# argumentcomputer/multi-stark

Hardware: NVIDIA B200
Metric: lde_merkle_gelem_per_s (higher is better)
Workload: dtype u64

## Files before the change

multi_stark_b200/csrc/fri.cu:

```cuda
#include "capi_common.hpp"
#include "mmcs.hpp"
#include "blake3.cuh"
#include <algorithm>
#include <cstring>
#include <memory>

namespace msg {

__device__ __forceinline__ u64 fp_inv_d(u64 x) {
    auto sqn = [](u64 v, int n) { for (int i = 0; i < n; i++) v = gl::mul(v, v); return v; };
    u64 t2 = gl::mul(sqn(x, 1), x);
    u64 t4 = gl::mul(sqn(t2, 2), t2);
    u64 t8 = gl::mul(sqn(t4, 4), t4);
    u64 t16 = gl::mul(sqn(t8, 8), t8);
    u64 t24 = gl::mul(sqn(t16, 8), t8);
    u64 t28 = gl::mul(sqn(t24, 4), t4);
    u64 t30 = gl::mul(sqn(t28, 2), t2);
    u64 t31 = gl::mul(sqn(t30, 1), x);
    u64 a = sqn(t31, 1);
    u64 b = gl::mul(a, x);
    return gl::mul(sqn(a, 32), b);
}
__device__ __forceinline__ gl::e2 e2_inverse_d(gl::e2 x) {
    u64 norm = gl::sub(gl::sqr(x.a), gl::mul7(gl::sqr(x.b)));
    u64 ni = fp_inv_d(norm);
    return gl::e2_make(gl::mul(x.a, ni), gl::mul(gl::neg(x.b), ni));
}

constexpr int kInvPerThread = 8;
__global__ void __launch_bounds__(256) k_inv_denoms(u64* invden, u32 log_h, gl::e2 z, gl::PowTable xtab, u64 row0, u64 len) {
    const u64 H = len;
    u64 i0 = ((u64)blockIdx.x * blockDim.x + threadIdx.x) * kInvPerThread;
    if (i0 >= H) return;
    const int cnt = (int)min((u64)kInvPerThread, H - i0);
    u64 va[kInvPerThread];
    gl::e2 pref[kInvPerThread];
    gl::e2 acc = gl::e2_make(1, 0);
#pragma unroll
    for (int k = 0; k < kInvPerThread; k++) {
        pref[k] = acc;
        va[k] = 0;
        if (k < cnt) {
            u64 x = gl::pow_lookup(xtab, gl::rev_bits((u32)(row0 + i0 + k), log_h));
            va[k] = gl::sub(z.a, x);
            acc = gl::e2_mul(acc, gl::e2_make(va[k], z.b));
        }
    }
    gl::e2 inv = e2_inverse_d(acc);
#pragma unroll
    for (int k = kInvPerThread - 1; k >= 0; k--) {
        if (k < cnt) {
            gl::e2 r = gl::e2_mul(inv, pref[k]);
            inv = gl::e2_mul(inv, gl::e2_make(va[k], z.b));
            invden[2 * (i0 + k)] = r.a;
            invden[2 * (i0 + k) + 1] = r.b;
        }
    }
}

constexpr int kMaxPts = 4;
struct BaryParams {
    const u64* M;
    const u64* invden[kMaxPts];
    u64* partial;
    u64 h;
    u32 w, c0, wc;
    u32 rows_per_step, tile_rows;
};
__host__ __device__ __forceinline__ size_t bary_dd_offset(u32 tile_rows, u32 wc) { return ((size_t)tile_rows * wc + 1) & ~(size_t)1; }
template <int NPTS>
__global__ void __launch_bounds__(256) k_bary_partial(BaryParams p) {
    extern __shared__ __align__(16) u64 sm_b[];
    const u32 t = threadIdx.x;
    const u32 TR = p.tile_rows, wc = p.wc;
    u64* tile = sm_b;
    ulonglong2* dd = reinterpret_cast<ulonglong2*>(sm_b + bary_dd_offset(TR, wc));
    const u32 active = p.rows_per_step * wc;
    const u32 c = t % wc, lane_row = t / wc;
    gl::Acc160 acc[2 * NPTS];
#pragma unroll
    for (int k = 0; k < 2 * NPTS; k++) acc[k] = gl::acc_zero();
// ... 897 lines not shown
```

multi_stark_b200/csrc/gl.cuh:

```cuda
#pragma once
#include <cstdint>
#include <cuda_runtime.h>

typedef unsigned long long u64;
typedef unsigned int u32;

#define GLD_P 0xFFFFFFFF00000001ull
#define GLD_EPS 0xFFFFFFFFull

namespace gl {


__device__ __forceinline__ u64 pack(u32 lo, u32 hi) { return ((u64)hi << 32) | lo; }

__device__ __forceinline__ u64 canon(u64 x) {
    u32 x0 = (u32)x, x1 = (u32)(x >> 32), r0, r1;
    asm("{\n\t"
        ".reg .u32 t, k;\n\t"
        "add.cc.u32 t, %2, 0xffffffff;\n\t"
        "addc.cc.u32 t, %3, 0;\n\t"
        "addc.u32 k, 0, 0;\n\t"
        "neg.s32 k, k;\n\t"
        "add.cc.u32 %0, %2, k;\n\t"
        "addc.u32 %1, %3, 0;\n\t"
// ... 39 lines not shown

__device__ __forceinline__ u64 reduce128_lazy(u64 lo, u64 hi) {
    u32 l0 = (u32)lo, l1 = (u32)(lo >> 32), hl = (u32)hi, hh = (u32)(hi >> 32), r0, r1;
    asm("{\n\t"
        ".reg .u32 m, k, t0, t1;\n\t"
        "sub.cc.u32 %0, %2, %5;\n\t"
        "subc.cc.u32 %1, %3, 0;\n\t"
        "subc.u32 m, 0, 0;\n\t"
        "sub.cc.u32 %0, %0, m;\n\t"
        "subc.u32 %1, %1, 0;\n\t"
        "sub.cc.u32 t0, 0, %4;\n\t"
        "subc.u32 t1, %4, 0;\n\t"
        "add.cc.u32 %0, %0, t0;\n\t"
        "addc.cc.u32 %1, %1, t1;\n\t"
        "addc.u32 k, 0, 0;\n\t"
        "neg.s32 k, k;\n\t"
        "add.cc.u32 %0, %0, k;\n\t"
        "addc.u32 %1, %1, 0;\n\t"
        "}"
        : "=&r"(r0), "=&r"(r1)
        : "r"(l0), "r"(l1), "r"(hl), "r"(hh));
    return pack(r0, r1);
}
namespace gf {
__device__ __forceinline__ u64 reduce128(u64 lo, u64 hi);
}
__device__ __forceinline__ u64 mul(u64 a, u64 b) {
    unsigned __int128 pr = (unsigned __int128)a * b;
    return gf::reduce128((u64)pr, (u64)(pr >> 64));
}
__device__ __forceinline__ u64 mul_lazy(u64 a, u64 b) { return reduce128_lazy(a * b, __umul64hi(a, b)); }
__device__ __forceinline__ u64 sqr(u64 a) { return mul(a, a); }

__device__ __forceinline__ u64 pow(u64 a, u64 e) {
    u64 acc = 1;
    while (e) {
        if (e & 1) acc = mul(acc, a);
        a = sqr(a);
        e >>= 1;
    }
    return acc;
}
__device__ __forceinline__ u64 inv(u64 a) { return pow(a, GLD_P - 2); }
__device__ __forceinline__ u64 halve(u64 a) { return (a & 1) ? (a >> 1) + (GLD_P >> 1) + 1 : a >> 1; }

namespace gf {
__device__ __forceinline__ u64 sub(u64 a, u64 b) { return sub_lazy(a, b); }
__device__ __forceinline__ u64 add(u64 a, u64 b) { return sub_lazy(a, GLD_P - b); }
__device__ __forceinline__ u64 reduce128(u64 lo, u64 hi) {
    u32 l0 = (u32)lo, l1 = (u32)(lo >> 32), h0 = (u32)hi, h1 = (u32)(hi >> 32);
    u64 r;
    asm("{\n\t"
        ".reg .u32 t0, t1, m, k, z, r0, r1;\n\t"
        ".reg .u64 rr;\n\t"
        "sub.cc.u32 t0, %1, %4;\n\t"
        "subc.cc.u32 t1, %2, 0;\n\t"
        "subc.u32 m, 0, 0;\n\t"
        "sub.cc.u32 t0, t0, m;\n\t"
        "subc.u32 t1, t1, 0;\n\t"
        "mad.lo.cc.u32 r0, %3, 0xffffffff, t0;\n\t"
        "madc.hi.cc.u32 r1, %3, 0xffffffff, t1;\n\t"
        "addc.u32 k, 0, 0;\n\t"
        "mov.b64 rr, {r0, r1};\n\t"
        "mad.wide.u32 rr, k, 0xffffffff, rr;\n\t"
        "mov.b64 {r0, r1}, rr;\n\t"
        "add.cc.u32 z, r0, 0xffffffff;\n\t"
        "addc.cc.u32 z, r1, 0;\n\t"
        "addc.u32 k, 0, 0;\n\t"
        "mad.wide.u32 %0, k, 0xffffffff, rr;\n\t"
        "}"
        : "=l"(r)
        : "r"(l0), "r"(l1), "r"(h0), "r"(h1));
    return r;
}
__device__ __forceinline__ u64 mul(u64 a, u64 b) {
    unsigned __int128 pr = (unsigned __int128)a * b;
// ... 36 lines not shown
        "mad.lo.cc.u32 %1, %5, %8, %1;\n\t"
        "madc.hi.cc.u32 %2, %5, %8, %2;\n\t"
        "addc.cc.u32 %3, %3, 0;\n\t"
        "addc.u32 %4, %4, 0;\n\t"
        "mad.lo.cc.u32 %1, %6, %7, %1;\n\t"
        "madc.hi.cc.u32 %2, %6, %7, %2;\n\t"
        "addc.cc.u32 %3, %3, 0;\n\t"
        "addc.u32 %4, %4, 0;\n\t"
        "}"
        : "+r"(s.l0), "+r"(s.l1), "+r"(s.l2), "+r"(s.l3), "+r"(s.l4)
        : "r"(a0), "r"(a1), "r"(b0), "r"(b1));
}
__device__ __forceinline__ u64 acc_reduce(const Acc160& s) {
    u64 r = gf::reduce128(pack(s.l0, s.l1), pack(s.l2, s.l3));
    return sub_lazy(r, (u64)s.l4 << 32);
}

struct e2 {
    u64 a, b;
};
__device__ __forceinline__ e2 e2_make(u64 a, u64 b) { e2 r; r.a = a; r.b = b; return r; }
__device__ __forceinline__ e2 e2_add(e2 x, e2 y) { return e2_make(add(x.a, y.a), add(x.b, y.b)); }
__device__ __forceinline__ e2 e2_sub(e2 x, e2 y) { return e2_make(sub(x.a, y.a), sub(x.b, y.b)); }
__device__ __forceinline__ u64 mul7(u64 x) {
    u64 x2 = add(x, x), x4 = add(x2, x2);
    return sub(add(x4, x4), x);
}
__device__ __forceinline__ e2 e2_mul(e2 x, e2 y) {
    u64 v0 = mul(x.a, y.a), v1 = mul(x.b, y.b);
    u64 cross = sub(sub(mul(add(x.a, x.b), add(y.a, y.b)), v0), v1);
    return e2_make(add(v0, mul7(v1)), cross);
}
__device__ __forceinline__ e2 e2_mul_base(e2 x, u64 s) { return e2_make(mul(x.a, s), mul(x.b, s)); }
__device__ __forceinline__ e2 e2_inv(e2 x) {
    u64 norm = sub(sqr(x.a), mul7(sqr(x.b)));
    u64 ni = inv(norm);
    return e2_make(mul(x.a, ni), mul(neg(x.b), ni));
}

struct PowTable {
    const u64* lo;
    const u64* hi;
    u32 h1;
};
__device__ __forceinline__ u64 pow_lookup(const PowTable& t, u64 e) {
    return mul(__ldg(t.hi + (e >> t.h1)), __ldg(t.lo + (e & ((1ull << t.h1) - 1))));
}

__device__ __forceinline__ u32 rev_bits(u32 x, u32 bits) { return bits ? (__brev(x) >> (32 - bits)) : 0u; }

}
```

multi_stark_b200/csrc/quotient.cu:

```cuda
#include "capi_common.hpp"
#include <cstdio>
#include <cstdlib>
#include "../host/blake3_host.hpp"
#include <cstring>
#include "mmcs.hpp"
#include "lowering.hpp"
#include <algorithm>
#include <cstring>

namespace msg {

}

struct msgpu_program {
    msg::Ctx* ctx = nullptr;
    msg::Instr* d_full = nullptr;
    msg::Instr* d_prefix = nullptr;
    u32 n_full = 0, n_prefix = 0, slots_full = 0, slots_prefix = 0;
    u32 n_zeros = 0, n_lookups = 0, n_args = 0;
    u32* d_zero_slots = nullptr;
    u32 *d_mult_full = nullptr, *d_args_full = nullptr;
    u32 *d_mult_prefix = nullptr, *d_args_prefix = nullptr;
    u32* d_arg_off = nullptr;
    u32 pre_width = 0, main_width = 0, stage2_width = 0;
    std::vector<void*> owned;
};

namespace msg {

__device__ __forceinline__ gl::e2 e2_mul_k(gl::e2 x, gl::e2 y) { return gl::e2_mul(x, y); }

__device__ __forceinline__ u64 fp_inv(u64 x) {
    auto sqn = [](u64 v, int n) { for (int i = 0; i < n; i++) v = gl::mul(v, v); return v; };
    u64 t2 = gl::mul(sqn(x, 1), x);
    u64 t4 = gl::mul(sqn(t2, 2), t2);
    u64 t8 = gl::mul(sqn(t4, 4), t4);
    u64 t16 = gl::mul(sqn(t8, 8), t8);
    u64 t24 = gl::mul(sqn(t16, 8), t8);
    u64 t28 = gl::mul(sqn(t24, 4), t4);
    u64 t30 = gl::mul(sqn(t28, 2), t2);
    u64 t31 = gl::mul(sqn(t30, 1), x);
    u64 a = sqn(t31, 1);
    u64 b = gl::mul(a, x);
    return gl::mul(sqn(a, 32), b);
}
__device__ __forceinline__ gl::e2 e2_inverse(gl::e2 x) {
    u64 norm = gl::sub(gl::sqr(x.a), gl::mul7(gl::sqr(x.b)));
    u64 ni = fp_inv(norm);
    return gl::e2_make(gl::mul(x.a, ni), gl::mul(gl::neg(x.b), ni));
}

struct RowCtx {
    const u64* rows[3][2];
    const u64* publics;
    u64 first, last, trans;
};

constexpr int kInterpThreads = 128;
constexpr int kSmemSlotsMax = 128;
template <int NSLOT, bool SMEM>
struct Slots;
template <int NSLOT>
struct Slots<NSLOT, false> {
    u64 v[NSLOT];
    __device__ __forceinline__ Slots() {}
    __device__ __forceinline__ u64& operator[](u32 k) { return v[k]; }
};
template <int NSLOT>
struct Slots<NSLOT, true> {
    u64* base;
    __device__ __forceinline__ Slots() {
        extern __shared__ u64 sm_slots[];
        base = sm_slots + threadIdx.x;
    }
    __device__ __forceinline__ u64& operator[](u32 k) { return base[(size_t)k * kInterpThreads]; }
};
template <int NSLOT>
constexpr size_t slots_smem_bytes() { return NSLOT <= kSmemSlotsMax ? (size_t)NSLOT * kInterpThreads * 8 : 0; }

struct NoRoots {
    __device__ __forceinline__ void operator()(u32, u64) const {}
};
template <int NSLOT, class S, class Root = NoRoots>
// ... 29 lines not shown
        }
        slots[dst] = v;
    }
}

struct SelParams {
    gl::PowTable xtab;
    const u64* zh;
    u64 g_inv;
    u64* first;
    u64* last;
    u32 log_nq, log_q;
};
constexpr int kSelPerThread = 4;
__global__ void __launch_bounds__(256) k_selectors(SelParams p) {
    const u64 nq = 1ull << p.log_nq;
    u64 s0 = ((u64)blockIdx.x * blockDim.x + threadIdx.x) * kSelPerThread;
    if (s0 >= nq) return;
    u64 den[2 * kSelPerThread], pref[2 * kSelPerThread], zh[kSelPerThread];
    int cnt = 0;
#pragma unroll
    for (int k = 0; k < kSelPerThread; k++) {
        u64 s = s0 + k;
        if (s >= nq) break;
        u64 i = gl::rev_bits((u32)s, p.log_nq);
        u64 x = gl::pow_lookup(p.xtab, i);
        den[2 * k] = gl::sub(x, 1);
        den[2 * k + 1] = gl::sub(x, p.g_inv);
        zh[k] = p.zh[i & ((1ull << p.log_q) - 1)];
        cnt = k + 1;
    }
    u64 acc = 1;
    for (int k = 0; k < 2 * cnt; k++) { pref[k] = acc; acc = gl::mul(acc, den[k]); }
    u64 inv = fp_inv(acc);
    for (int k = 2 * cnt; k-- > 0;) {
        u64 d = den[k];
        den[k] = gl::mul(inv, pref[k]);
        inv = gl::mul(inv, d);
    }
    for (int k = 0; k < cnt; k++) {
        p.first[s0 + k] = gl::mul(zh[k], den[2 * k]);
        p.last[s0 + k] = gl::mul(zh[k], den[2 * k + 1]);
    }
}

struct QuotParams {
    const Instr* prog;
    const u32* zero_slots;
    const u32 *lk_mult, *lk_argoff, *lk_args;
    const u64 *pre, *s1, *s2;
    const u64* apow;
    const u64 *sel_first, *sel_last, *inv_zh;
    u64* out;
    const u64 *pre_n, *s1_n, *s2_n;
    u32 wn[3], cn[3];
    u64 row0, n_local, next_row0;
    u32 out_stored;
    gl::PowTable xtab;
    u64 publics[8];
    u64 delta[2];
    u64 g_inv;
    u32 n_instr, n_zeros, n_lookups;
    u32 wpre, w1, w2;
    u32 log_nq, log_q;
};

template <int NSLOT>
// ... 37 lines not shown
        fold(gl::add(gl::sub(s2n[1], s2c[1]), inj.b));
    } else {
        for (u32 j = 0; j < p.n_lookups; j++) {
            gl::e2 source = gl::e2_make(s2c[2 * j], s2c[2 * j + 1]);
            gl::e2 target = j + 1 < p.n_lookups ? gl::e2_make(s2c[2 * j + 2], s2c[2 * j + 3])
                                                : gl::e2_make(gl::add(s2n[0], inj.a), gl::add(s2n[1], inj.b));
            gl::e2 f = gl::e2_make(0, 0);
            for (u32 k = p.lk_argoff[j + 1]; k-- > p.lk_argoff[j];) {
                f = gl::e2_mul(f, gamma);
                f.a = gl::add(f.a, slots[p.lk_args[k]]);
            }
            gl::e2 c = gl::e2_mul(gl::e2_add(f, beta), gl::e2_sub(target, source));
            fold(gl::sub(c.a, slots[p.lk_mult[j]]));
            fold(c.b);
        }
    }
    const u64 iv = p.inv_zh[i & ((1ull << p.log_q) - 1)];
    const u64 o = p.out_stored ? sl : i;
    p.out[2 * o] = gl::mul(gl::acc_reduce(fa0), iv);
    p.out[2 * o + 1] = gl::mul(gl::acc_reduce(fa1), iv);
}

__global__ void k_quotient_slices(const u64* S, u64* out, u32 log_big, u32 log_n, u32 d, const u64* weights) {
    const u64 big = 1ull << log_big, n = 1ull << log_n, q = big >> log_n;
    u64 t = (u64)blockIdx.x * blockDim.x + threadIdx.x;
    if (t >= big) return;
    u64 r = t / q, k = t % q;
    u64 j = k * n + r;
    u64 src = gl::rev_bits((u32)((big - j) & (big - 1)), log_big);
    u64 w = weights[k];
    for (u32 c = 0; c < d; c++) out[r * (q * d) + k * d + c] = gl::mul(S[src * d + c], w);
}

struct MsgParams {
    const Instr* prog;
    const u32 *lk_mult, *lk_argoff, *lk_args;
    const u64 *pre, *main;
    u64* msgs;
    u64* mults;
    u64 rows;
    u64 beta[2], gamma[2];
    u32 n_instr, n_lookups, wpre, wmain;
};
template <int NSLOT>
__global__ void __launch_bounds__(128) k_lookup_messages(MsgParams p) {
    const u64 r = (u64)blockIdx.x * blockDim.x + threadIdx.x;
    if (r >= p.rows) return;
    const u64 rn = r + 1 == p.rows ? 0 : r + 1;
    RowCtx cx;
    cx.rows[0][0] = p.pre + r * p.wpre;
    cx.rows[0][1] = p.pre + rn * p.wpre;
    cx.rows[1][0] = p.main + r * p.wmain;
    cx.rows[1][1] = p.main + rn * p.wmain;
    cx.rows[2][0] = cx.rows[2][1] = nullptr;
    cx.publics = nullptr;
    cx.first = r == 0;
    cx.last = r + 1 == p.rows;
    cx.trans = r + 1 != p.rows;
    Slots<NSLOT, (NSLOT <= kSmemSlotsMax)> slots;
    run_program<NSLOT>(p.prog, p.n_instr, slots, cx);
    const gl::e2 beta = gl::e2_make(p.beta[0], p.beta[1]), gamma = gl::e2_make(p.gamma[0], p.gamma[1]);
    for (u32 j = 0; j < p.n_lookups; j++) {
        gl::e2 f = gl::e2_make(0, 0);
        for (u32 k = p.lk_argoff[j + 1]; k-- > p.lk_argoff[j];) {
            f = gl::e2_mul(f, gamma);
            f.a = gl::add(f.a, slots[p.lk_args[k]]);
        }
        f = gl::e2_add(f, beta);
        u64 idx = r * p.n_lookups + j;
        p.msgs[2 * idx] = f.a;
        p.msgs[2 * idx + 1] = f.b;
        p.mults[idx] = slots[p.lk_mult[j]];
    }
}

constexpr int kScanPerThread = 8;
constexpr int kScanThreads = 256;
constexpr int kScanPerBlock = kScanPerThread * kScanThreads;

__device__ __forceinline__ gl::e2 block_sum(gl::e2 v, gl::e2* sm) {
    for (int off = 16; off > 0; off >>= 1) {
        v.a = gl::add(v.a, __shfl_down_sync(0xffffffffu, v.a, off));
        v.b = gl::add(v.b, __shfl_down_sync(0xffffffffu, v.b, off));
    }
    int lane = threadIdx.x & 31, wid = threadIdx.x >> 5;
    if (lane == 0) sm[wid] = v;
    __syncthreads();
    gl::e2 r = gl::e2_make(0, 0);
    if (threadIdx.x == 0)
        for (int w = 0; w < (int)(blockDim.x >> 5); w++) r = gl::e2_add(r, sm[w]);
    return r;
}

__global__ void __launch_bounds__(kScanThreads) k_terms_and_block_sums(u64* msgs, const u64* mults, u64 total, u64* block_sums) {
    __shared__ gl::e2 sm[kScanThreads / 32];
    u64 i0 = ((u64)blockIdx.x * kScanThreads + threadIdx.x) * kScanPerThread;
    gl::e2 pref[kScanPerThread];
    const int cnt = (int)min((u64)kScanPerThread, total > i0 ? total - i0 : 0);
    gl::e2 acc = gl::e2_make(1, 0);
#pragma unroll
    for (int k = 0; k < kScanPerThread; k++) {
        pref[k] = acc;
        if (k < cnt) acc = gl::e2_mul(acc, gl::e2_make(msgs[2 * (i0 + k)], msgs[2 * (i0 + k) + 1]));
    }
    gl::e2 inv = cnt ? e2_inverse(acc) : acc;
    gl::e2 sum = gl::e2_make(0, 0);
#pragma unroll
    for (int k = kScanPerThread - 1; k >= 0; k--) {
        if (k < cnt) {
            gl::e2 x = gl::e2_make(msgs[2 * (i0 + k)], msgs[2 * (i0 + k) + 1]);
            gl::e2 xi = gl::e2_mul(inv, pref[k]);
            inv = gl::e2_mul(inv, x);
            gl::e2 term = gl::e2_mul_base(xi, mults[i0 + k]);
            msgs[2 * (i0 + k)] = term.a;
            msgs[2 * (i0 + k) + 1] = term.b;
            sum = gl::e2_add(sum, term);
        }
    }
    gl::e2 bs = block_sum(sum, sm);
    if (threadIdx.x == 0) { block_sums[2 * blockIdx.x] = bs.a; block_sums[2 * blockIdx.x + 1] = bs.b; }
}

__global__ void __launch_bounds__(1024) k_scan_block_sums(u64* block_sums, u64 nblocks) {
    __shared__ gl::e2 sm[1024];
    u64 per = (nblocks + blockDim.x - 1) / blockDim.x;
    u64 lo = (u64)threadIdx.x * per, hi = min(nblocks, lo + per);
    gl::e2 s = gl::e2_make(0, 0);
    for (u64 i = lo; i < hi; i++) s = gl::e2_add(s, gl::e2_make(block_sums[2 * i], block_sums[2 * i + 1]));
    sm[threadIdx.x] = s;
    __syncthreads();
    for (int off = 1; off < (int)blockDim.x; off <<= 1) {
        gl::e2 t = sm[threadIdx.x];
        if ((int)threadIdx.x >= off) t = gl::e2_add(t, sm[threadIdx.x - off]);
        __syncthreads();
        sm[threadIdx.x] = t;
        __syncthreads();
    }
    gl::e2 run = threadIdx.x ? sm[threadIdx.x - 1] : gl::e2_make(0, 0);
    for (u64 i = lo; i < hi; i++) {
        gl::e2 v = gl::e2_make(block_sums[2 * i], block_sums[2 * i + 1]);
        block_sums[2 * i] = run.a;
        block_sums[2 * i + 1] = run.b;
        run = gl::e2_add(run, v);
    }
    if (threadIdx.x == blockDim.x - 1) {
        gl::e2 tot = sm[blockDim.x - 1];
        block_sums[2 * nblocks] = tot.a;
        block_sums[2 * nblocks + 1] = tot.b;
    }
}

__global__ void __launch_bounds__(kScanThreads) k_scan_write(const u64* terms, u64 total, const u64* block_offsets, u64* out) {
    __shared__ gl::e2 sm[kScanThreads];
    u64 i0 = ((u64)blockIdx.x * kScanThreads + threadIdx.x) * kScanPerThread;
    gl::e2 v[kScanPerThread];
    gl::e2 s = gl::e2_make(0, 0);
    for (int k = 0; k < kScanPerThread; k++) {
        v[k] = i0 + k < total ? gl::e2_make(terms[2 * (i0 + k)], terms[2 * (i0 + k) + 1]) : gl::e2_make(0, 0);
        s = gl::e2_add(s, v[k]);
    }
    sm[threadIdx.x] = s;
    __syncthreads();
    for (int off = 1; off < kScanThreads; off <<= 1) {
        gl::e2 t = sm[threadIdx.x];
        if ((int)threadIdx.x >= off) t = gl::e2_add(t, sm[threadIdx.x - off]);
        __syncthreads();
        sm[threadIdx.x] = t;
        __syncthreads();
    }
    gl::e2 run = gl::e2_make(block_offsets[2 * blockIdx.x], block_offsets[2 * blockIdx.x + 1]);
    if (threadIdx.x) run = gl::e2_add(run, sm[threadIdx.x - 1]);
    for (int k = 0; k < kScanPerThread; k++) {
        if (i0 + k >= total) break;
        out[2 * (i0 + k)] = run.a;
        out[2 * (i0 + k) + 1] = run.b;
        run = gl::e2_add(run, v[k]);
    }
}

__global__ void __launch_bounds__(kScanThreads) k_claims(const u64* claims, u64 n_claims, u32 len, gl::e2 beta, gl::e2 gamma,
                                                         u64* partial) {
    __shared__ gl::e2 sm[kScanThreads / 32];
    u64 i0 = ((u64)blockIdx.x * kScanThreads + threadIdx.x) * kScanPerThread;
    const int cnt = (int)min((u64)kScanPerThread, n_claims > i0 ? n_claims - i0 : 0);
    gl::e2 v[kScanPerThread], pref[kScanPerThread];
    gl::e2 acc = gl::e2_make(1, 0);
#pragma unroll
    for (int k = 0; k < kScanPerThread; k++) {
        pref[k] = acc;
        v[k] = acc;
        if (k < cnt) {
            const u64* c = claims + (i0 + k) * len;
            gl::e2 f = gl::e2_make(0, 0);
            for (u32 a = len; a-- > 0;) {
                f = gl::e2_mul(f, gamma);
                f.a = gl::add(f.a, c[a]);
            }
            v[k] = gl::e2_add(f, beta);
            acc = gl::e2_mul(acc, v[k]);
        }
    }
    gl::e2 inv = cnt ? e2_inverse(acc) : acc;
    gl::e2 sum = gl::e2_make(0, 0);
#pragma unroll
    for (int k = kScanPerThread - 1; k >= 0; k--) {
        if (k < cnt) {
            sum = gl::e2_add(sum, gl::e2_mul(inv, pref[k]));
            inv = gl::e2_mul(inv, v[k]);
        }
    }
    gl::e2 bs = block_sum(sum, sm);
    if (threadIdx.x == 0) { partial[2 * blockIdx.x] = bs.a; partial[2 * blockIdx.x + 1] = bs.b; }
}

template <class T>
static T* upload_vec(Ctx& c, msgpu_program* prog, const std::vector<T>& v) {
    T* d = nullptr;
    MSG_CUDA(cudaMalloc(&d, std::max<size_t>(v.size(), 1) * sizeof(T)));
    prog->owned.push_back(d);
    if (!v.empty()) MSG_CUDA(cudaMemcpyAsync(d, v.data(), v.size() * sizeof(T), cudaMemcpyHostToDevice, c.stream));
    return d;
}

static msgpu_program* program_create(Ctx& c, const msgpu_graph_desc& g) {
    MSG_REQUIRE(g.lookup_prefix_len <= g.n_nodes, "program: lookup prefix longer than the node vector");
    MSG_REQUIRE(g.stage2_width == 2 * std::max<u32>(g.n_lookups, 1), "program: stage-2 width must be 2 * max(lookups, 1)");
    std::vector<u32> pin_lk, pin_all;
    u32 n_args = g.n_lookups ? g.lookup_arg_off[g.n_lookups] : 0;
    for (u32 j = 0; j < g.n_lookups; j++) pin_lk.push_back(g.lookup_mult[j]);
    for (u32 k = 0; k < n_args; k++) pin_lk.push_back(g.lookup_args[k]);
    pin_all = pin_lk;
    std::vector<u32> roots(g.zeros, g.zeros + g.n_zeros);
    for (u32 p : pin_lk) MSG_REQUIRE(p < g.lookup_prefix_len, "program: lookup node outside the prefix");
    Lowered full, prefix;
    try {
// ... 125 lines not shown
    *ptr = m.ptr;
}

}

using namespace msg;

struct msgpu_claims {
    Ctx* ctx;
    u64* d;
    u64 n, len;
    cudaEvent_t ready = nullptr;
};

namespace msg {
__global__ void __launch_bounds__(256) k_encode_claims(const u64* claims, u64 n_words, u32 len, uint8_t* msg) {
    u64 j = (u64)blockIdx.x * blockDim.x + threadIdx.x;
    if (j >= n_words) return;
    u64 claim = j / (len + 1);
    u32 k = (u32)(j % (len + 1));
    u64 v = k == 0 ? (u64)len : claims[claim * len + (k - 1)];
    uint8_t* o = msg + 8 * j;
#pragma unroll
    for (int b = 0; b < 8; b++) o[b] = (uint8_t)(v >> (8 * b));
}
}

static void claims_sum(Ctx& c, const u64* d_claims, u64 n_claims, u64 claim_len, const uint64_t* beta2, const uint64_t* gamma2,
                       uint64_t* out2) {
    StageScope ss(c, "stage2");
    out2[0] = out2[1] = 0;
    if (n_claims == 0) return;
    u64 nblocks = (n_claims + kScanPerBlock - 1) / kScanPerBlock;
    DevBuf part(c, nblocks * 16);
    {
        KLaunch kl(c, "k_claims");
        k_claims<<<(unsigned)nblocks, kScanThreads, 0, c.stream>>>(d_claims, n_claims, (u32)claim_len, gl::e2{beta2[0], beta2[1]},
                                                                   gl::e2{gamma2[0], gamma2[1]}, part.u());
    }
    MSG_CUDA(cudaGetLastError());
    std::vector<u64> hp(nblocks * 2);
    MSG_CUDA(cudaMemcpyAsync(hp.data(), part.p, nblocks * 16, cudaMemcpyDeviceToHost, c.stream));
    c.sync();
    msh::Fp2 acc;
    for (u64 b = 0; b < nblocks; b++) acc += msh::Fp2(msh::Fp(hp[2 * b]), msh::Fp(hp[2 * b + 1]));
    out2[0] = acc.c[0].v;
    out2[1] = acc.c[1].v;
}

extern "C" {

int msgpu_program_create(msgpu_ctx* h, const msgpu_graph_desc* desc, msgpu_program** out) {
    return guard([&] {
        MSG_REQUIRE(desc && out, "program_create: null argument");
        *out = program_create(h->c, *desc);
    });
}
void msgpu_program_free(msgpu_program* prog) {
    if (!prog) return;
    cudaStreamSynchronize(prog->ctx->stream);
    for (void* p : prog->owned) cudaFree(p);
    delete prog;
}

int msgpu_stage2_trace(msgpu_ctx* h, const msgpu_program* prog, const uint64_t* pre_dev, const uint64_t* main_dev,
                       uint64_t rows, const uint64_t* beta2, const uint64_t* gamma2, uint64_t* stage2_out_dev,
                       uint64_t* local_sum2) {
    return guard([&] {
        Ctx& c = h->c;
        StageScope ss(c, "stage2");
        MSG_REQUIRE(prog && stage2_out_dev && local_sum2, "stage2_trace: null argument");
        MSG_REQUIRE(main_dev || prog->n_lookups == 0, "stage2_trace: the main trace is needed to evaluate the lookups");
        MSG_REQUIRE(prog->pre_width == 0 || pre_dev, "stage2_trace: circuit has a preprocessed trace but none was given");
        local_sum2[0] = local_sum2[1] = 0;
        if (rows == 0) return;
        u32 L = prog->n_lookups;
        if (L == 0) {
            MSG_CUDA(cudaMemsetAsync(stage2_out_dev, 0, rows * 2 * 8, c.stream));
            return;
        }
        u64 total = rows * L;
        u64 nblocks = (total + kScanPerBlock - 1) / kScanPerBlock;
        DevBuf msgs(c, total * 16), mults(c, total * 8), bsums(c, (nblocks + 1) * 16);
        MsgParams mp{};
        mp.prog = prog->d_prefix;
        mp.n_instr = prog->n_prefix;
        mp.lk_mult = prog->d_mult_prefix;
        mp.lk_argoff = prog->d_arg_off;
        mp.lk_args = prog->d_args_prefix;
        mp.pre = (const u64*)pre_dev;
        mp.main = (const u64*)main_dev;
        mp.msgs = msgs.u();
        mp.mults = mults.u();
        mp.rows = rows;
        mp.beta[0] = beta2[0]; mp.beta[1] = beta2[1];
        mp.gamma[0] = gamma2[0]; mp.gamma[1] = gamma2[1];
        mp.n_lookups = L;
        mp.wpre = prog->pre_width;
        mp.wmain = prog->main_width;
        launch_by_slots(prog->slots_prefix, [&](auto ns) {
            KLaunch kl(c, "k_lookup_messages");
            constexpr int NS = decltype(ns)::value;
            constexpr size_t smem = slots_smem_bytes<NS>();
            if (smem > 48 * 1024) ensure_max_smem(k_lookup_messages<NS>, (int)smem);
            k_lookup_messages<NS><<<(unsigned)((rows + 127) / 128), kInterpThreads, smem, c.stream>>>(mp);
        });
        MSG_CUDA(cudaGetLastError());
        {
            KLaunch kl(c, "k_terms_and_block_sums");
            k_terms_and_block_sums<<<(unsigned)nblocks, kScanThreads, 0, c.stream>>>(msgs.u(), mults.u(), total, bsums.u());
        }
        MSG_CUDA(cudaGetLastError());
        {
            KLaunch kl(c, "k_scan_block_sums");
            k_scan_block_sums<<<1, 1024, 0, c.stream>>>(bsums.u(), nblocks);
        }
        MSG_CUDA(cudaGetLastError());
        {
            KLaunch kl(c, "k_scan_write");
            k_scan_write<<<(unsigned)nblocks, kScanThreads, 0, c.stream>>>(msgs.u(), total, bsums.u(), (u64*)stage2_out_dev);
        }
        MSG_CUDA(cudaGetLastError());
        MSG_CUDA(cudaMemcpyAsync(local_sum2, bsums.u() + 2 * nblocks, 16, cudaMemcpyDeviceToHost, c.stream));
        c.sync();
    });
}

int msgpu_claims_accumulator(msgpu_ctx* h, const uint64_t* claims, uint64_t n_claims, uint64_t claim_len,
                             const uint64_t* beta2, const uint64_t* gamma2, uint64_t* out2) {
    return guard([&] {
        Ctx& c = h->c;
        MSG_REQUIRE(claim_len < (1ull << 31), "claims: claim too long");
        DevBuf d(c, n_claims * std::max<u64>(claim_len, 1) * 8);
        if (claim_len && n_claims) MSG_CUDA(cudaMemcpyAsync(d.p, claims, n_claims * claim_len * 8, cudaMemcpyHostToDevice, c.stream));
        claims_sum(c, d.u(), n_claims, claim_len, beta2, gamma2, out2);
    });
}

static void claims_digest(Ctx& c, const u64* d_claims, u64 n_claims, u64 claim_len, const uint8_t* prefix, u64 prefix_len, uint8_t* digest32);

int msgpu_claims_upload(msgpu_ctx* h, const uint64_t* claims, uint64_t n_claims, uint64_t claim_len, const uint8_t* prefix,
                        uint64_t prefix_len, msgpu_claims** out, uint8_t* digest32) {
    return guard([&] {
        Ctx& c = h->c;
        MSG_REQUIRE(out && digest32 && claims && n_claims > 0 && claim_len > 0, "claims_upload: null or empty argument");
        MSG_REQUIRE(claim_len < (1ull << 31) && n_claims <= (~0ull) / 16 / (claim_len + 1), "claims_upload: too large");
        u64 n_vals = n_claims * claim_len;
        DevBuf d(c, n_vals * 8);
        MSG_CUDA(cudaMemcpyAsync(d.p, claims, n_vals * 8, cudaMemcpyHostToDevice, c.stream));
        claims_digest(c, d.u(), n_claims, claim_len, prefix, prefix_len, digest32);
        *out = new msgpu_claims{&c, (u64*)d.release(), n_claims, claim_len};
    });
}

int msgpu_claims_prefetch(msgpu_ctx* h, const uint64_t* claims, uint64_t n_claims, uint64_t claim_len, msgpu_claims** out) {
    return guard([&] {
        Ctx& c = h->c;
// ... 276 lines not shown
```

Before: 27.02.

## Fuse lookup messages and logup inverses, batch inversions across warps

Merges the lookup message kernel and the term/block-sum kernel into one k_logup_terms kernel. It takes the inverse through the base-field norm, with running products stored in the output buffer, so the msgs and mults temporaries go away. Field inversions are batched across a warp with shuffles, so one exponentiation serves 32 threads, with a zero flag for failures. It also rewrites the scan-write as a warp-shuffle scan over spans and unifies the inverse helpers. This adds recomputation of lookup fingerprints and a zero-check readback. The measured LDE/Merkle metric likely only touches k_inv_denoms, via the warp inverse.

After: 27.06, median of 6. Within noise of the previous version (+0.1%).

```diff
diff --git a/multi_stark_b200/csrc/fri.cu b/multi_stark_b200/csrc/fri.cu
--- a/multi_stark_b200/csrc/fri.cu
+++ b/multi_stark_b200/csrc/fri.cu
@@ -7,32 +7,11 @@
 
 namespace msg {
 
-__device__ __forceinline__ u64 fp_inv_d(u64 x) {
-    auto sqn = [](u64 v, int n) { for (int i = 0; i < n; i++) v = gl::mul(v, v); return v; };
-    u64 t2 = gl::mul(sqn(x, 1), x);
-    u64 t4 = gl::mul(sqn(t2, 2), t2);
-    u64 t8 = gl::mul(sqn(t4, 4), t4);
-    u64 t16 = gl::mul(sqn(t8, 8), t8);
-    u64 t24 = gl::mul(sqn(t16, 8), t8);
-    u64 t28 = gl::mul(sqn(t24, 4), t4);
-    u64 t30 = gl::mul(sqn(t28, 2), t2);
-    u64 t31 = gl::mul(sqn(t30, 1), x);
-    u64 a = sqn(t31, 1);
-    u64 b = gl::mul(a, x);
-    return gl::mul(sqn(a, 32), b);
-}
-__device__ __forceinline__ gl::e2 e2_inverse_d(gl::e2 x) {
-    u64 norm = gl::sub(gl::sqr(x.a), gl::mul7(gl::sqr(x.b)));
-    u64 ni = fp_inv_d(norm);
-    return gl::e2_make(gl::mul(x.a, ni), gl::mul(gl::neg(x.b), ni));
-}
-
 constexpr int kInvPerThread = 8;
 __global__ void __launch_bounds__(256) k_inv_denoms(u64* invden, u32 log_h, gl::e2 z, gl::PowTable xtab, u64 row0, u64 len) {
     const u64 H = len;
     u64 i0 = ((u64)blockIdx.x * blockDim.x + threadIdx.x) * kInvPerThread;
-    if (i0 >= H) return;
-    const int cnt = (int)min((u64)kInvPerThread, H - i0);
+    const int cnt = (int)min((u64)kInvPerThread, H > i0 ? H - i0 : 0);
     u64 va[kInvPerThread];
     gl::e2 pref[kInvPerThread];
     gl::e2 acc = gl::e2_make(1, 0);
@@ -46,7 +25,8 @@
             acc = gl::e2_mul(acc, gl::e2_make(va[k], z.b));
         }
     }
-    gl::e2 inv = e2_inverse_d(acc);
+    bool any_zero;
+    gl::e2 inv = gl::e2_inv_warp(acc, any_zero);
 #pragma unroll
     for (int k = kInvPerThread - 1; k >= 0; k--) {
         if (k < cnt) {
diff --git a/multi_stark_b200/csrc/gl.cuh b/multi_stark_b200/csrc/gl.cuh
--- a/multi_stark_b200/csrc/gl.cuh
+++ b/multi_stark_b200/csrc/gl.cuh
@@ -95,16 +95,20 @@
 __device__ __forceinline__ u64 mul_lazy(u64 a, u64 b) { return reduce128_lazy(a * b, __umul64hi(a, b)); }
 __device__ __forceinline__ u64 sqr(u64 a) { return mul(a, a); }
 
-__device__ __forceinline__ u64 pow(u64 a, u64 e) {
-    u64 acc = 1;
-    while (e) {
-        if (e & 1) acc = mul(acc, a);
-        a = sqr(a);
-        e >>= 1;
-    }
-    return acc;
-}
-__device__ __forceinline__ u64 inv(u64 a) { return pow(a, GLD_P - 2); }
+__device__ __forceinline__ u64 inv(u64 x) {
+    auto sqn = [](u64 v, int n) { for (int i = 0; i < n; i++) v = mul(v, v); return v; };
+    u64 t2 = mul(sqn(x, 1), x);
+    u64 t4 = mul(sqn(t2, 2), t2);
+    u64 t8 = mul(sqn(t4, 4), t4);
+    u64 t16 = mul(sqn(t8, 8), t8);
+    u64 t24 = mul(sqn(t16, 8), t8);
+    u64 t28 = mul(sqn(t24, 4), t4);
+    u64 t30 = mul(sqn(t28, 2), t2);
+    u64 t31 = mul(sqn(t30, 1), x);
+    u64 a = sqn(t31, 1);
+    u64 b = mul(a, x);
+    return mul(sqn(a, 32), b);
+}
 __device__ __forceinline__ u64 halve(u64 a) { return (a & 1) ? (a >> 1) + (GLD_P >> 1) + 1 : a >> 1; }
 
 namespace gf {
@@ -207,9 +211,28 @@
     return e2_make(add(v0, mul7(v1)), cross);
 }
 __device__ __forceinline__ e2 e2_mul_base(e2 x, u64 s) { return e2_make(mul(x.a, s), mul(x.b, s)); }
+__device__ __forceinline__ u64 e2_norm(e2 x) { return sub(sqr(x.a), mul7(sqr(x.b))); }
 __device__ __forceinline__ e2 e2_inv(e2 x) {
-    u64 norm = sub(sqr(x.a), mul7(sqr(x.b)));
-    u64 ni = inv(norm);
+    u64 ni = inv(e2_norm(x));
+    return e2_make(mul(x.a, ni), mul(neg(x.b), ni));
+}
+
+__device__ __forceinline__ u64 inv_warp(u64 x, bool& any_zero) {
+    u64 sib[5];
+    u64 g = x;
+#pragma unroll
+    for (int k = 0; k < 5; k++) {
+        sib[k] = __shfl_xor_sync(0xffffffffu, g, 1 << k);
+        g = mul(g, sib[k]);
+    }
+    any_zero = g == 0;
+    u64 gi = inv(g);
+#pragma unroll
+    for (int k = 4; k >= 0; k--) gi = mul(gi, sib[k]);
+    return gi;
+}
+__device__ __forceinline__ e2 e2_inv_warp(e2 x, bool& any_zero) {
+    const u64 ni = inv_warp(e2_norm(x), any_zero);
     return e2_make(mul(x.a, ni), mul(neg(x.b), ni));
 }
 
diff --git a/multi_stark_b200/csrc/quotient.cu b/multi_stark_b200/csrc/quotient.cu
--- a/multi_stark_b200/csrc/quotient.cu
+++ b/multi_stark_b200/csrc/quotient.cu
@@ -29,26 +29,6 @@
 namespace msg {
 
 __device__ __forceinline__ gl::e2 e2_mul_k(gl::e2 x, gl::e2 y) { return gl::e2_mul(x, y); }
-
-__device__ __forceinline__ u64 fp_inv(u64 x) {
-    auto sqn = [](u64 v, int n) { for (int i = 0; i < n; i++) v = gl::mul(v, v); return v; };
-    u64 t2 = gl::mul(sqn(x, 1), x);
-    u64 t4 = gl::mul(sqn(t2, 2), t2);
-    u64 t8 = gl::mul(sqn(t4, 4), t4);
-    u64 t16 = gl::mul(sqn(t8, 8), t8);
-    u64 t24 = gl::mul(sqn(t16, 8), t8);
-    u64 t28 = gl::mul(sqn(t24, 4), t4);
-    u64 t30 = gl::mul(sqn(t28, 2), t2);
-    u64 t31 = gl::mul(sqn(t30, 1), x);
-    u64 a = sqn(t31, 1);
-    u64 b = gl::mul(a, x);
-    return gl::mul(sqn(a, 32), b);
-}
-__device__ __forceinline__ gl::e2 e2_inverse(gl::e2 x) {
-    u64 norm = gl::sub(gl::sqr(x.a), gl::mul7(gl::sqr(x.b)));
-    u64 ni = fp_inv(norm);
-    return gl::e2_make(gl::mul(x.a, ni), gl::mul(gl::neg(x.b), ni));
-}
 
 struct RowCtx {
     const u64* rows[3][2];
@@ -144,7 +124,7 @@
     }
     u64 acc = 1;
     for (int k = 0; k < 2 * cnt; k++) { pref[k] = acc; acc = gl::mul(acc, den[k]); }
-    u64 inv = fp_inv(acc);
+    u64 inv = gl::inv(acc);
     for (int k = 2 * cnt; k-- > 0;) {
         u64 d = den[k];
         den[k] = gl::mul(inv, pref[k]);
@@ -248,48 +228,6 @@
     for (u32 c = 0; c < d; c++) out[r * (q * d) + k * d + c] = gl::mul(S[src * d + c], w);
 }
 
-struct MsgParams {
-    const Instr* prog;
-    const u32 *lk_mult, *lk_argoff, *lk_args;
-    const u64 *pre, *main;
-    u64* msgs;
-    u64* mults;
-    u64 rows;
-    u64 beta[2], gamma[2];
-    u32 n_instr, n_lookups, wpre, wmain;
-};
-template <int NSLOT>
-__global__ void __launch_bounds__(128) k_lookup_messages(MsgParams p) {
-    const u64 r = (u64)blockIdx.x * blockDim.x + threadIdx.x;
-    if (r >= p.rows) return;
-    const u64 rn = r + 1 == p.rows ? 0 : r + 1;
-    RowCtx cx;
-    cx.rows[0][0] = p.pre + r * p.wpre;
-    cx.rows[0][1] = p.pre + rn * p.wpre;
-    cx.rows[1][0] = p.main + r * p.wmain;
-    cx.rows[1][1] = p.main + rn * p.wmain;
-    cx.rows[2][0] = cx.rows[2][1] = nullptr;
-    cx.publics = nullptr;
-    cx.first = r == 0;
-    cx.last = r + 1 == p.rows;
-    cx.trans = r + 1 != p.rows;
-    Slots<NSLOT, (NSLOT <= kSmemSlotsMax)> slots;
-    run_program<NSLOT>(p.prog, p.n_instr, slots, cx);
-    const gl::e2 beta = gl::e2_make(p.beta[0], p.beta[1]), gamma = gl::e2_make(p.gamma[0], p.gamma[1]);
-    for (u32 j = 0; j < p.n_lookups; j++) {
-        gl::e2 f = gl::e2_make(0, 0);
-        for (u32 k = p.lk_argoff[j + 1]; k-- > p.lk_argoff[j];) {
-            f = gl::e2_mul(f, gamma);
-            f.a = gl::add(f.a, slots[p.lk_args[k]]);
-        }
-        f = gl::e2_add(f, beta);
-        u64 idx = r * p.n_lookups + j;
-        p.msgs[2 * idx] = f.a;
-        p.msgs[2 * idx + 1] = f.b;
-        p.mults[idx] = slots[p.lk_mult[j]];
-    }
-}
-
 constexpr int kScanPerThread = 8;
 constexpr int kScanThreads = 256;
 constexpr int kScanPerBlock = kScanPerThread * kScanThreads;
@@ -308,33 +246,84 @@
     return r;
 }
 
-__global__ void __launch_bounds__(kScanThreads) k_terms_and_block_sums(u64* msgs, const u64* mults, u64 total, u64* block_sums) {
-    __shared__ gl::e2 sm[kScanThreads / 32];
-    u64 i0 = ((u64)blockIdx.x * kScanThreads + threadIdx.x) * kScanPerThread;
-    gl::e2 pref[kScanPerThread];
-    const int cnt = (int)min((u64)kScanPerThread, total > i0 ? total - i0 : 0);
-    gl::e2 acc = gl::e2_make(1, 0);
-#pragma unroll
-    for (int k = 0; k < kScanPerThread; k++) {
-        pref[k] = acc;
-        if (k < cnt) acc = gl::e2_mul(acc, gl::e2_make(msgs[2 * (i0 + k)], msgs[2 * (i0 + k) + 1]));
-    }
-    gl::e2 inv = cnt ? e2_inverse(acc) : acc;
+template <class Arg>
+__device__ __forceinline__ gl::e2 fingerprint(u32 n, Arg arg, gl::e2 gamma) {
+    if (n == 0) return gl::e2_make(0, 0);
+    const u64 last = gl::add(0, arg(n - 1));
+    if (n == 1) return gl::e2_make(last, 0);
+    gl::e2 f = gl::e2_mul_base(gamma, last);
+    f.a = gl::add(f.a, arg(n - 2));
+    for (u32 k = n - 2; k-- > 0;) {
+        f = gl::e2_mul(f, gamma);
+        f.a = gl::add(f.a, arg(k));
+    }
+    return f;
+}
+
+template <class S>
+__device__ __forceinline__ gl::e2 lookup_message(S& slots, const u32* __restrict__ argoff, const u32* __restrict__ args, u32 j,
+                                                 gl::e2 beta, gl::e2 gamma) {
+    const u32 k0 = argoff[j];
+    return gl::e2_add(fingerprint(argoff[j + 1] - k0, [&](u32 k) { return slots[args[k0 + k]]; }, gamma), beta);
+}
+
+struct LogupParams {
+    const Instr* prog;
+    const u32 *lk_mult, *lk_argoff, *lk_args;
+    const u64 *pre, *main;
+    u64* out;
+    u64* block_sums;
+    u32* zero_flag;
+    u64 rows;
+    u64 beta[2], gamma[2];
+    u32 n_instr, n_lookups, wpre, wmain;
+};
+template <int NSLOT>
+__global__ void __launch_bounds__(kInterpThreads) k_logup_terms(LogupParams p) {
+    __shared__ gl::e2 sm[kInterpThreads / 32];
+    const u64 r = (u64)blockIdx.x * blockDim.x + threadIdx.x;
+    const bool active = r < p.rows;
+    const u32 L = p.n_lookups;
+    const gl::e2 beta = gl::e2_make(p.beta[0], p.beta[1]), gamma = gl::e2_make(p.gamma[0], p.gamma[1]);
+    ulonglong2* o = reinterpret_cast<ulonglong2*>(p.out) + r * L;
+    Slots<NSLOT, (NSLOT <= kSmemSlotsMax)> slots;
+    u64 acc = 1;
+    if (active) {
+        const u64 rn = r + 1 == p.rows ? 0 : r + 1;
+        RowCtx cx;
+        cx.rows[0][0] = p.pre + r * p.wpre;
+        cx.rows[0][1] = p.pre + rn * p.wpre;
+        cx.rows[1][0] = p.main + r * p.wmain;
+        cx.rows[1][1] = p.main + rn * p.wmain;
+        cx.rows[2][0] = cx.rows[2][1] = nullptr;
+        cx.publics = nullptr;
+        cx.first = r == 0;
+        cx.last = r + 1 == p.rows;
+        cx.trans = r + 1 != p.rows;
+        run_program<NSLOT>(p.prog, p.n_instr, slots, cx);
+        for (u32 j = 0; j < L; j++) {
+            const u64 n = gl::e2_norm(lookup_message(slots, p.lk_argoff, p.lk_args, j, beta, gamma));
+            o[j] = make_ulonglong2(acc, n);
+            acc = gl::mul(acc, n);
+        }
+    }
+    bool any_zero;
+    u64 inv = gl::inv_warp(acc, any_zero);
+    if (any_zero && (threadIdx.x & 31) == 0) *p.zero_flag = 1;
     gl::e2 sum = gl::e2_make(0, 0);
-#pragma unroll
-    for (int k = kScanPerThread - 1; k >= 0; k--) {
-        if (k < cnt) {
-            gl::e2 x = gl::e2_make(msgs[2 * (i0 + k)], msgs[2 * (i0 + k) + 1]);
-            gl::e2 xi = gl::e2_mul(inv, pref[k]);
-            inv = gl::e2_mul(inv, x);
-            gl::e2 term = gl::e2_mul_base(xi, mults[i0 + k]);
-            msgs[2 * (i0 + k)] = term.a;
-            msgs[2 * (i0 + k) + 1] = term.b;
-            sum = gl::e2_add(sum, term);
+    if (active) {
+        for (u32 j = L; j-- > 0;) {
+            const ulonglong2 c = o[j];
+            const u64 s = gl::mul(gl::mul(inv, c.x), slots[p.lk_mult[j]]);
+            inv = gl::mul(inv, c.y);
+            const gl::e2 m = lookup_message(slots, p.lk_argoff, p.lk_args, j, beta, gamma);
+            const gl::e2 t = gl::e2_make(gl::mul(m.a, s), gl::mul(gl::neg(m.b), s));
+            o[j] = make_ulonglong2(t.a, t.b);
+            sum = gl::e2_add(sum, t);
         }
     }
     gl::e2 bs = block_sum(sum, sm);
-    if (threadIdx.x == 0) { block_sums[2 * blockIdx.x] = bs.a; block_sums[2 * blockIdx.x + 1] = bs.b; }
+    if (threadIdx.x == 0) { p.block_sums[2 * blockIdx.x] = bs.a; p.block_sums[2 * blockIdx.x + 1] = bs.b; }
 }
 
 __global__ void __launch_bounds__(1024) k_scan_block_sums(u64* block_sums, u64 nblocks) {
@@ -366,36 +355,56 @@
     }
 }
 
-__global__ void __launch_bounds__(kScanThreads) k_scan_write(const u64* terms, u64 total, const u64* block_offsets, u64* out) {
-    __shared__ gl::e2 sm[kScanThreads];
-    u64 i0 = ((u64)blockIdx.x * kScanThreads + threadIdx.x) * kScanPerThread;
-    gl::e2 v[kScanPerThread];
-    gl::e2 s = gl::e2_make(0, 0);
-    for (int k = 0; k < kScanPerThread; k++) {
-        v[k] = i0 + k < total ? gl::e2_make(terms[2 * (i0 + k)], terms[2 * (i0 + k) + 1]) : gl::e2_make(0, 0);
-        s = gl::e2_add(s, v[k]);
-    }
-    sm[threadIdx.x] = s;
-    __syncthreads();
-    for (int off = 1; off < kScanThreads; off <<= 1) {
-        gl::e2 t = sm[threadIdx.x];
-        if ((int)threadIdx.x >= off) t = gl::e2_add(t, sm[threadIdx.x - off]);
+__global__ void __launch_bounds__(kScanThreads) k_scan_write(u64* terms, u64 total, u64 span, const u64* block_offsets) {
+    constexpr int kWarps = kScanThreads / 32;
+    __shared__ gl::e2 wsum[kWarps];
+    ulonglong2* t2 = reinterpret_cast<ulonglong2*>(terms);
+    const int lane = threadIdx.x & 31, warp = threadIdx.x >> 5;
+    const u64 lo = (u64)blockIdx.x * span, hi = min(total, lo + span);
+    gl::e2 run = gl::e2_make(block_offsets[2 * blockIdx.x], block_offsets[2 * blockIdx.x + 1]);
+    for (u64 t0 = lo; t0 < hi; t0 += kScanPerBlock) {
+        const u64 w0 = t0 + (u64)warp * (32 * kScanPerThread);
+        gl::e2 x[kScanPerThread];
+        gl::e2 carry = gl::e2_make(0, 0);
+#pragma unroll
+        for (int k = 0; k < kScanPerThread; k++) {
+            const u64 i = w0 + 32 * k + lane;
+            gl::e2 v = gl::e2_make(0, 0);
+            if (i < hi) {
+                const ulonglong2 w = t2[i];
+                v = gl::e2_make(w.x, w.y);
+            }
+            gl::e2 s = v;
+#pragma unroll
+            for (int off = 1; off < 32; off <<= 1) {
+                const u64 a = __shfl_up_sync(0xffffffffu, s.a, off), b = __shfl_up_sync(0xffffffffu, s.b, off);
+                if (lane >= off) s = gl::e2_add(s, gl::e2_make(a, b));
+            }
+            x[k] = gl::e2_add(carry, gl::e2_sub(s, v));
+            carry = gl::e2_add(carry, gl::e2_make(__shfl_sync(0xffffffffu, s.a, 31), __shfl_sync(0xffffffffu, s.b, 31)));
+        }
+        if (lane == 0) wsum[warp] = carry;
         __syncthreads();
-        sm[threadIdx.x] = t;
+        gl::e2 base = run;
+#pragma unroll
+        for (int w = 0; w < kWarps; w++) {
+            if (w == warp) base = run;
+            run = gl::e2_add(run, wsum[w]);
+        }
+#pragma unroll
+        for (int k = 0; k < kScanPerThread; k++) {
+            const u64 i = w0 + 32 * k + lane;
+            if (i < hi) {
+                const gl::e2 y = gl::e2_add(base, x[k]);
+                t2[i] = make_ulonglong2(y.a, y.b);
+            }
+        }
         __syncthreads();
     }
-    gl::e2 run = gl::e2_make(block_offsets[2 * blockIdx.x], block_offsets[2 * blockIdx.x + 1]);
-    if (threadIdx.x) run = gl::e2_add(run, sm[threadIdx.x - 1]);
-    for (int k = 0; k < kScanPerThread; k++) {
-        if (i0 + k >= total) break;
-        out[2 * (i0 + k)] = run.a;
-        out[2 * (i0 + k) + 1] = run.b;
-        run = gl::e2_add(run, v[k]);
-    }
 }
 
 __global__ void __launch_bounds__(kScanThreads) k_claims(const u64* claims, u64 n_claims, u32 len, gl::e2 beta, gl::e2 gamma,
-                                                         u64* partial) {
+                                                         u64* partial, u32* zero_flag) {
     __shared__ gl::e2 sm[kScanThreads / 32];
     u64 i0 = ((u64)blockIdx.x * kScanThreads + threadIdx.x) * kScanPerThread;
     const int cnt = (int)min((u64)kScanPerThread, n_claims > i0 ? n_claims - i0 : 0);
@@ -407,16 +416,13 @@
         v[k] = acc;
         if (k < cnt) {
             const u64* c = claims + (i0 + k) * len;
-            gl::e2 f = gl::e2_make(0, 0);
-            for (u32 a = len; a-- > 0;) {
-                f = gl::e2_mul(f, gamma);
-                f.a = gl::add(f.a, c[a]);
-            }
-            v[k] = gl::e2_add(f, beta);
+            v[k] = gl::e2_add(fingerprint(len, [&](u32 a) { return c[a]; }, gamma), beta);
             acc = gl::e2_mul(acc, v[k]);
         }
     }
-    gl::e2 inv = cnt ? e2_inverse(acc) : acc;
+    bool any_zero;
+    gl::e2 inv = gl::e2_inv_warp(acc, any_zero);
+    if (any_zero && (threadIdx.x & 31) == 0) *zero_flag = 1;
     gl::e2 sum = gl::e2_make(0, 0);
 #pragma unroll
     for (int k = kScanPerThread - 1; k >= 0; k--) {
@@ -608,16 +614,19 @@
     out2[0] = out2[1] = 0;
     if (n_claims == 0) return;
     u64 nblocks = (n_claims + kScanPerBlock - 1) / kScanPerBlock;
-    DevBuf part(c, nblocks * 16);
+    DevBuf part(c, nblocks * 16 + 8);
+    u32* zero_flag = (u32*)(part.u() + 2 * nblocks);
+    MSG_CUDA(cudaMemsetAsync(zero_flag, 0, 8, c.stream));
     {
         KLaunch kl(c, "k_claims");
         k_claims<<<(unsigned)nblocks, kScanThreads, 0, c.stream>>>(d_claims, n_claims, (u32)claim_len, gl::e2{beta2[0], beta2[1]},
-                                                                   gl::e2{gamma2[0], gamma2[1]}, part.u());
+                                                                   gl::e2{gamma2[0], gamma2[1]}, part.u(), zero_flag);
     }
     MSG_CUDA(cudaGetLastError());
-    std::vector<u64> hp(nblocks * 2);
-    MSG_CUDA(cudaMemcpyAsync(hp.data(), part.p, nblocks * 16, cudaMemcpyDeviceToHost, c.stream));
+    std::vector<u64> hp(nblocks * 2 + 1);
+    MSG_CUDA(cudaMemcpyAsync(hp.data(), part.p, nblocks * 16 + 8, cudaMemcpyDeviceToHost, c.stream));
     c.sync();
+    MSG_REQUIRE(hp[2 * nblocks] == 0, "claims: beta + fingerprint of a claim is zero (no inverse)");
     msh::Fp2 acc;
     for (u64 b = 0; b < nblocks; b++) acc += msh::Fp2(msh::Fp(hp[2 * b]), msh::Fp(hp[2 * b + 1]));
     out2[0] = acc.c[0].v;
@@ -655,37 +664,35 @@
             MSG_CUDA(cudaMemsetAsync(stage2_out_dev, 0, rows * 2 * 8, c.stream));
             return;
         }
-        u64 total = rows * L;
-        u64 nblocks = (total + kScanPerBlock - 1) / kScanPerBlock;
-        DevBuf msgs(c, total * 16), mults(c, total * 8), bsums(c, (nblocks + 1) * 16);
-        MsgParams mp{};
-        mp.prog = prog->d_prefix;
-        mp.n_instr = prog->n_prefix;
-        mp.lk_mult = prog->d_mult_prefix;
-        mp.lk_argoff = prog->d_arg_off;
-        mp.lk_args = prog->d_args_prefix;
-        mp.pre = (const u64*)pre_dev;
-        mp.main = (const u64*)main_dev;
-        mp.msgs = msgs.u();
-        mp.mults = mults.u();
-        mp.rows = rows;
-        mp.beta[0] = beta2[0]; mp.beta[1] = beta2[1];
-        mp.gamma[0] = gamma2[0]; mp.gamma[1] = gamma2[1];
-        mp.n_lookups = L;
-        mp.wpre = prog->pre_width;
-        mp.wmain = prog->main_width;
+        u64 total = rows * L, span = (u64)kInterpThreads * L;
+        u64 nblocks = (rows + kInterpThreads - 1) / kInterpThreads;
+        DevBuf bsums(c, (nblocks + 1) * 16 + 8);
+        u32* zero_flag = (u32*)(bsums.u() + 2 * (nblocks + 1));
+        MSG_CUDA(cudaMemsetAsync(zero_flag, 0, 8, c.stream));
+        LogupParams lp{};
+        lp.prog = prog->d_prefix;
+        lp.n_instr = prog->n_prefix;
+        lp.lk_mult = prog->d_mult_prefix;
+        lp.lk_argoff = prog->d_arg_off;
+        lp.lk_args = prog->d_args_prefix;
+        lp.pre = (const u64*)pre_dev;
+        lp.main = (const u64*)main_dev;
+        lp.out = (u64*)stage2_out_dev;
+        lp.block_sums = bsums.u();
+        lp.zero_flag = zero_flag;
+        lp.rows = rows;
+        lp.beta[0] = beta2[0]; lp.beta[1] = beta2[1];
+        lp.gamma[0] = gamma2[0]; lp.gamma[1] = gamma2[1];
+        lp.n_lookups = L;
+        lp.wpre = prog->pre_width;
+        lp.wmain = prog->main_width;
         launch_by_slots(prog->slots_prefix, [&](auto ns) {
-            KLaunch kl(c, "k_lookup_messages");
+            KLaunch kl(c, "k_logup_terms");
             constexpr int NS = decltype(ns)::value;
             constexpr size_t smem = slots_smem_bytes<NS>();
-            if (smem > 48 * 1024) ensure_max_smem(k_lookup_messages<NS>, (int)smem);
-            k_lookup_messages<NS><<<(unsigned)((rows + 127) / 128), kInterpThreads, smem, c.stream>>>(mp);
+            if (smem > 48 * 1024) ensure_max_smem(k_logup_terms<NS>, (int)smem);
+            k_logup_terms<NS><<<(unsigned)nblocks, kInterpThreads, smem, c.stream>>>(lp);
         });
-        MSG_CUDA(cudaGetLastError());
-        {
-            KLaunch kl(c, "k_terms_and_block_sums");
-            k_terms_and_block_sums<<<(unsigned)nblocks, kScanThreads, 0, c.stream>>>(msgs.u(), mults.u(), total, bsums.u());
-        }
         MSG_CUDA(cudaGetLastError());
         {
             KLaunch kl(c, "k_scan_block_sums");
@@ -694,11 +701,15 @@
         MSG_CUDA(cudaGetLastError());
         {
             KLaunch kl(c, "k_scan_write");
-            k_scan_write<<<(unsigned)nblocks, kScanThreads, 0, c.stream>>>(msgs.u(), total, bsums.u(), (u64*)stage2_out_dev);
+            k_scan_write<<<(unsigned)nblocks, kScanThreads, 0, c.stream>>>((u64*)stage2_out_dev, total, span, bsums.u());
         }
         MSG_CUDA(cudaGetLastError());
-        MSG_CUDA(cudaMemcpyAsync(local_sum2, bsums.u() + 2 * nblocks, 16, cudaMemcpyDeviceToHost, c.stream));
+        u64 tail[3];
+        MSG_CUDA(cudaMemcpyAsync(tail, bsums.u() + 2 * nblocks, 24, cudaMemcpyDeviceToHost, c.stream));
         c.sync();
+        MSG_REQUIRE(tail[2] == 0, "stage2_trace: a lookup message (beta + fingerprint) is zero (no inverse)");
+        local_sum2[0] = tail[0];
+        local_sum2[1] = tail[1];
     });
 }
 
```
